# zendesk/min-tfs-client

Hardware: AMD Instinct MI355X
Metric: predict_req_per_s (higher is better)
Workload: dtype fp32; 1 GPU; model=identity-echo[resnet50], global_batch=32, parallelism=dp1, pipeline=4, encoding=turbo, grpc_impl=native, copy_mode=1, streaming=auto, transport=unix, servers_per_rank=1, gpu=True

## Files before the change

min_tfs_client_amd/ops/csrc/grpc_transport.cpp:

```cpp
#include <pybind11/eval.h>
#include <pybind11/functional.h>
#include <pybind11/pybind11.h>
#include <pybind11/stl.h>
#include <torch/extension.h>

#include <c10/hip/HIPCachingAllocator.h>
#include <c10/hip/HIPGuard.h>
#include <c10/hip/HIPStream.h>

#include <algorithm>
#include <atomic>
#include <chrono>
#include <condition_variable>
#include <cstring>
#include <deque>
#include <map>
#include <memory>
#include <mutex>
#include <set>
#include <string>
#include <thread>
#include <unordered_map>
#include <vector>

#include "h2core.h"
#include "hpack.h"
#include "staging.h"
#include "wire.h"

namespace py = pybind11;

namespace {

using h2::Buf;
using h2::Conn;
using h2::ConnError;
using h2::FrameHeader;

struct WireRegion {
  size_t offset;
  size_t nbytes;
  uintptr_t ptr;
  bool device;
};

void write_message_with_regions(Conn& conn, uint32_t stream,
                                const uint8_t* buf, size_t len,
                                const std::vector<WireRegion>& regions,
                                bool end_stream) {
  h2::DataMessageWriter w(conn, stream, len, end_stream);
  size_t pos = 0;
  for (const auto& r : regions) {
    if (r.offset < pos || r.nbytes > len || r.offset > len - r.nbytes)
      throw ConnError("bad streaming region");
    if (r.offset > pos) w.write(buf + pos, r.offset - pos);
    if (!r.device) {
      w.write(reinterpret_cast<const uint8_t*>(r.ptr), r.nbytes);
    } else {
      mi355x_staging::Lease lease;
      lease.ctx->d2h(reinterpret_cast<const void*>(r.ptr), r.nbytes,
                     [&w](const void* chunk, size_t n) {
                       w.write(static_cast<const uint8_t*>(chunk), n);
                     });
    }
    pos = r.offset + r.nbytes;
  }
  if (pos < len) w.write(buf + pos, len - pos);
  w.finish();
}

bool extract_streaming_reply(py::handle result,
                             std::unique_ptr<py::buffer_info>* info,
                             const uint8_t** buf, size_t* len,
                             std::vector<WireRegion>* regions) {
  if (!py::hasattr(result, "_wire_regions")) return false;
  py::object buffer = result.attr("buffer");
  *info = std::make_unique<py::buffer_info>(py::buffer(buffer).request());
  *buf = static_cast<const uint8_t*>((*info)->ptr);
  *len = size_t((*info)->size) * size_t((*info)->itemsize);
// ... 1306 lines not shown
    }
  }
};


class GrpcChannel {
 public:
  explicit GrpcChannel(const std::string& target,
                       std::string authority = "")
      : authority_(std::move(authority)) {
    if (authority_.empty()) {
      authority_ = target.rfind("unix:", 0) == 0 ? "localhost" : target;
    }
    int fd = h2::connect_target(target);
    conn_ = std::make_shared<Conn>(fd);
    h2::write_all(fd, reinterpret_cast<const uint8_t*>(h2::kPreface),
                  h2::kPrefaceLen);
    conn_->send_initial_settings();
    reader_ = std::thread([this] { reader_loop(); });
  }

  ~GrpcChannel() { close(); }

  void close() {
    bool was = closed_.exchange(true);
    if (was) return;
    conn_->mark_broken("channel closed");
    if (reader_.joinable()) reader_.join();
    fail_all_pending(GRPC_UNAVAILABLE, "channel closed");
  }

  uint32_t begin_stream(const std::string& path, double timeout_s) {
    auto p = std::make_shared<Pending>();
    uint32_t id;
    {
      std::unique_lock<std::mutex> lk(mu_);
      cv_.wait(lk, [&] {
        int64_t maxs;
        {
          std::lock_guard<std::mutex> flk(conn_->fc_mu);
          maxs = conn_->peer_max_streams;
          if (conn_->broken) return true;
        }
        return maxs < 0 || int64_t(pending_.size()) < maxs;
      });
      {
        std::lock_guard<std::mutex> flk(conn_->fc_mu);
        if (conn_->broken)
          throw RpcCallError(GRPC_UNAVAILABLE,
                             "channel broken: " + conn_->broken_why);
      }
      id = next_stream_;
      next_stream_ += 2;
      pending_[id] = p;
      conn_->open_send_stream(id);
      std::string block = make_request_headers(path, timeout_s);
      try {
        conn_->send_headers(id, block, false);
      } catch (const std::exception& e) {
        pending_.erase(id);
        conn_->close_send_stream(id);
        throw RpcCallError(GRPC_UNAVAILABLE, e.what());
      }
    }
    return id;
  }

  uint32_t start_call(const std::string& path, const uint8_t* data,
                      size_t len, double timeout_s) {
    uint32_t id = begin_stream(path, timeout_s);
    try {
      conn_->send_data_message(id, data, len, true);
    } catch (const std::exception& e) {
      std::lock_guard<std::mutex> lk(mu_);
      pending_.erase(id);
      conn_->close_send_stream(id);
      throw RpcCallError(GRPC_UNAVAILABLE, e.what());
    }
    return id;
  }

  hipStream_t device_stream(int dev) {
    return ProspectStreams::instance().get(dev);
  }

  uint32_t start_call_streaming(const std::string& path, const uint8_t* buf,
                                size_t len,
                                const std::vector<WireRegion>& regions,
                                double timeout_s, int parse_device = -1) {
    uint32_t id = begin_stream(path, timeout_s);
    if (parse_device >= 0) {
      hipStream_t ds = device_stream(parse_device);
      if (ds != nullptr) {
        auto p = find_pending(id);
        if (p) {
          std::lock_guard<std::mutex> lk(p->m);
          p->dparse.enabled = true;
          p->dparse.device = parse_device;
          p->dparse.stream = ds;
        }
      }
    }
    try {
      write_message_with_regions(*conn_, id, buf, len, regions, true);
    } catch (const std::exception& e) {
      std::lock_guard<std::mutex> lk(mu_);
// ... 21 lines not shown
    }
    auto quiesce = [&] {
      std::lock_guard<std::mutex> lk(p->m);
      if (p->dparse.enabled && p->dparse.stream != nullptr)
        (void)hipStreamSynchronize(p->dparse.stream);
    };
    std::unique_lock<std::mutex> lk(p->m);
    bool ok = true;
    if (timeout_s > 0) {
      ok = p->cv.wait_for(lk, std::chrono::duration<double>(timeout_s),
                          [&] { return p->done; });
    } else {
      p->cv.wait(lk, [&] { return p->done; });
    }
    if (!ok) {
      lk.unlock();
      quiesce();
      {
        std::lock_guard<std::mutex> glk(mu_);
        pending_.erase(id);
      }
      try {
        conn_->send_rst_stream(id, 8 );
      } catch (...) {
      }
      conn_->close_send_stream(id);
      cv_.notify_all();
      throw RpcCallError(GRPC_DEADLINE_EXCEEDED, "Deadline Exceeded");
    }
    ParsedResult r;
    r.resp = std::move(p->body.msg);
    int status = p->grpc_status;
    std::string msg = p->message;
    bool parsed = p->dparse.enabled && !p->dparse.failed && p->dparse.done;
    if (parsed) r.outs = std::move(p->dparse.outs);
    bool need_sync = p->dparse.enabled && p->dparse.stream != nullptr;
    hipStream_t ds = p->dparse.stream;
    lk.unlock();
    if (need_sync && hipStreamSynchronize(ds) != hipSuccess) parsed = false;
    if (parsed) record_consumer_stream(r.outs, r.outs.empty() ? 0 :
        r.outs.front().second.get_device());
    {
      std::lock_guard<std::mutex> glk(mu_);
      pending_.erase(id);
    }
    conn_->close_send_stream(id);
    cv_.notify_all();
    if (status != GRPC_OK)
      throw RpcCallError(status < 0 ? GRPC_INTERNAL : status, msg);
    r.parsed_ok = parsed;
    return r;
  }

  Buf wait(uint32_t id, double timeout_s) {
    std::shared_ptr<Pending> p;
    {
      std::lock_guard<std::mutex> lk(mu_);
      auto it = pending_.find(id);
      if (it == pending_.end())
        throw RpcCallError(GRPC_INTERNAL, "unknown call handle");
      p = it->second;
    }
    std::unique_lock<std::mutex> lk(p->m);
    bool ok = true;
    if (timeout_s > 0) {
      ok = p->cv.wait_for(lk, std::chrono::duration<double>(timeout_s),
                          [&] { return p->done; });
    } else {
      p->cv.wait(lk, [&] { return p->done; });
    }
    if (!ok) {
      lk.unlock();
      {
        std::lock_guard<std::mutex> glk(mu_);
        pending_.erase(id);
      }
      try {
        conn_->send_rst_stream(id, 8 );
      } catch (...) {
      }
      conn_->close_send_stream(id);
      cv_.notify_all();
      throw RpcCallError(GRPC_DEADLINE_EXCEEDED, "Deadline Exceeded");
    }
    Buf resp = std::move(p->body.msg);
    int status = p->grpc_status;
    std::string msg = p->message;
    lk.unlock();
    {
      std::lock_guard<std::mutex> glk(mu_);
      pending_.erase(id);
    }
    conn_->close_send_stream(id);
    cv_.notify_all();
    if (status != GRPC_OK)
      throw RpcCallError(status < 0 ? GRPC_INTERNAL : status, msg);
    return resp;
  }

 private:
  struct Pending {
    std::mutex m;
    std::condition_variable cv;
    bool done = false;
    int grpc_status = -1;
    std::string message;
    std::vector<h2::Header> resp_headers;
    HeaderBlock hb;
    MsgAssembly body;
    DeviceParse dparse;
  };

  std::shared_ptr<Conn> conn_;
  std::thread reader_;
  std::string authority_;
  std::atomic<bool> closed_{false};
  std::mutex mu_;
  std::condition_variable cv_;
  std::unordered_map<uint32_t, std::shared_ptr<Pending>> pending_;
  uint32_t next_stream_ = 1;

  std::string make_request_headers(const std::string& path,
                                   double timeout_s) {
    h2::HpackEncoder enc;
    std::string block;
    enc.add_indexed(&block, 3);
    enc.add_indexed(&block, 6);
    enc.add_literal(&block, 4, path, true);
    enc.add_literal(&block, 1, authority_);
    enc.add_literal(&block, "te", "trailers");
    enc.add_literal(&block, 31, "application/grpc");
    if (timeout_s > 0) {
      long ms = long(timeout_s * 1000.0);
      if (ms < 1) ms = 1;
      enc.add_literal(&block, "grpc-timeout", std::to_string(ms) + "m");
    }
    return block;
  }

  std::shared_ptr<Pending> find_pending(uint32_t id) {
    std::lock_guard<std::mutex> lk(mu_);
    auto it = pending_.find(id);
    return it == pending_.end() ? nullptr : it->second;
  }

  void complete(const std::shared_ptr<Pending>& p, int status,
                std::string msg) {
    {
      std::lock_guard<std::mutex> lk(p->m);
      if (p->done) return;
      p->grpc_status = status;
      p->message = std::move(msg);
      p->done = true;
    }
    p->cv.notify_all();
  }

  void fail_all_pending(int status, const std::string& msg) {
    std::vector<std::shared_ptr<Pending>> ps;
    {
      std::lock_guard<std::mutex> lk(mu_);
      for (auto& kv : pending_) ps.push_back(kv.second);
    }
    for (auto& p : ps) complete(p, status, msg);
    cv_.notify_all();
  }

  void process_headers(uint32_t stream, const std::shared_ptr<Pending>& p,
                       std::vector<h2::Header>&& headers, bool end_stream) {
    const std::string* gs = find_header(headers, "grpc-status");
    if (gs != nullptr || end_stream) {
      int status = GRPC_UNKNOWN;
      std::string msg = "missing grpc-status";
// ... 85 lines not shown
            break;
          }
          case h2::F_SETTINGS: {
            if (fh.flags & h2::FL_ACK) {
              h2::discard(conn_->fd, fh.length);
            } else {
              std::vector<uint8_t> payload(fh.length);
              if (fh.length)
                h2::read_full(conn_->fd, payload.data(), fh.length);
              conn_->apply_peer_settings(payload.data(), fh.length);
              conn_->send_settings_ack();
            }
            break;
          }
          case h2::F_PING: {
            uint8_t opaque[8];
            if (fh.length != 8) throw ConnError("bad PING");
            h2::read_full(conn_->fd, opaque, 8);
            if (!(fh.flags & h2::FL_ACK)) conn_->send_ping_ack(opaque);
            break;
          }
          case h2::F_WINDOW_UPDATE: {
            uint8_t buf4[4];
            if (fh.length != 4) throw ConnError("bad WINDOW_UPDATE");
            h2::read_full(conn_->fd, buf4, 4);
            conn_->apply_window_update(fh.stream,
                                       h2::be32(buf4) & 0x7fffffff);
            break;
          }
          case h2::F_RST_STREAM: {
            uint8_t buf4[4];
            if (fh.length != 4) throw ConnError("bad RST_STREAM");
            h2::read_full(conn_->fd, buf4, 4);
            auto p = find_pending(fh.stream);
            if (p)
              complete(p, GRPC_UNAVAILABLE,
                       "stream reset by server (http2 code " +
                           std::to_string(h2::be32(buf4)) + ")");
            break;
          }
          case h2::F_GOAWAY:
          default:
            h2::discard(conn_->fd, fh.length);
            break;
        }
      }
    } catch (const std::exception& e) {
      conn_->mark_broken(e.what());
      fail_all_pending(GRPC_UNAVAILABLE,
                       std::string("connection lost: ") + e.what());
    }
  }
};

}


PYBIND11_MODULE(_transport, m) {
  m.doc() = "Native gRPC (HTTP/2) transport for the MI355X serving stack";

  py::class_<OwnedBuf>(m, "OwnedBuf", py::buffer_protocol())
      .def_buffer([](OwnedBuf& b) -> py::buffer_info {
        return py::buffer_info(b.buf.p, 1,
                               py::format_descriptor<uint8_t>::format(),
                               1, {py::ssize_t(b.buf.len)}, {py::ssize_t(1)},
                               true );
      })
      .def("__len__", [](const OwnedBuf& b) { return b.buf.len; })
      .def("tobytes", [](const OwnedBuf& b) {
        return py::bytes(reinterpret_cast<const char*>(b.buf.p), b.buf.len);
      });

  static py::object rpc_error_cls = [&m]() {
    py::dict ns;
    py::exec(R"(
class NativeRpcError(Exception):
    """gRPC call failure from the native transport (code_int, details)."""
    def __init__(self, code, details):
        super().__init__(code, details)
        self.code_int = code
        self.details = details
)",
             ns, ns);
    py::object cls = ns["NativeRpcError"];
    m.attr("NativeRpcError") = cls;
    return cls;
  }();

  py::register_exception_translator([](std::exception_ptr ep) {
    try {
      if (ep) std::rethrow_exception(ep);
    } catch (const RpcCallError& e) {
      py::object exc = rpc_error_cls(e.code, e.what());
      PyErr_SetObject(rpc_error_cls.ptr(), exc.ptr());
    }
  });

  py::class_<GrpcServer>(m, "GrpcServer")
      .def(py::init<std::string, int>(), py::arg("address"),
           py::arg("workers") = 8)
      .def("start", &GrpcServer::start,
           py::call_guard<py::gil_scoped_release>())
      .def("register_handler", &GrpcServer::register_handler,
           py::arg("path"), py::arg("fn"))
      .def("register_handler_parsed", &GrpcServer::register_handler_parsed,
           py::arg("path"), py::arg("fn"), py::arg("device"),
// ... 107 lines not shown
            if (r.parsed_ok) {
              py::dict d;
              for (auto& kv : r.outs) d[py::str(kv.first)] = kv.second;
              outs = std::move(d);
            }
            return py::make_tuple(outs, OwnedBuf(std::move(r.resp)));
          },
          py::arg("id"), py::arg("timeout") = 0.0,
          "wait() for calls started with parse_device >= 0: returns "
          "({name: device tensor} | None, raw buf).")
      .def(
          "start_streaming",
          [](GrpcChannel& ch, const std::string& path, py::buffer data,
             py::list region_list, double timeout, int parse_device) {
            py::buffer_info info = data.request();
            const uint8_t* ptr = static_cast<const uint8_t*>(info.ptr);
            size_t len = size_t(info.size) * size_t(info.itemsize);
            std::vector<WireRegion> regions;
            regions.reserve(py::len(region_list));
            for (auto item : region_list) {
              auto t = py::reinterpret_borrow<py::tuple>(item);
              regions.push_back(WireRegion{
                  t[0].cast<size_t>(), t[1].cast<size_t>(),
                  uintptr_t(t[2].cast<uint64_t>()), t[3].cast<bool>()});
            }
            py::gil_scoped_release release;
            return ch.start_call_streaming(path, ptr, len, regions,
                                           timeout, parse_device);
          },
          py::arg("path"), py::arg("data"), py::arg("regions"),
          py::arg("timeout") = 0.0, py::arg("parse_device") = -1,
          "Streaming-region variant of start(); the send completes before "
          "this returns (region memory may be released), the response is "
          "collected with wait().")
      .def(
          "start",
          [](GrpcChannel& ch, const std::string& path, py::buffer data,
             double timeout) {
            py::buffer_info info = data.request();
            const uint8_t* ptr = static_cast<const uint8_t*>(info.ptr);
            size_t len = size_t(info.size) * size_t(info.itemsize);
            py::gil_scoped_release release;
            return ch.start_call(path, ptr, len, timeout);
          },
          py::arg("path"), py::arg("data"), py::arg("timeout") = 0.0)
      .def(
          "wait",
          [](GrpcChannel& ch, uint32_t id, double timeout) {
            py::gil_scoped_release release;
            Buf resp = ch.wait(id, timeout);
            return OwnedBuf(std::move(resp));
          },
          py::arg("id"), py::arg("timeout") = 0.0)
      .def("close", &GrpcChannel::close,
           py::call_guard<py::gil_scoped_release>());
}
```

min_tfs_client_amd/ops/csrc/native.cpp:

```cpp

#include <torch/extension.h>

#include <algorithm>
#include <atomic>
#include <chrono>
#include <cstring>
#include <string>
#include <thread>
#include <vector>

#include "wire.h"

namespace py = pybind11;

namespace mi355x {
at::Tensor cast_op(const at::Tensor& in, at::ScalarType out_dtype);
at::Tensor nchw_to_nhwc(const at::Tensor& in, at::ScalarType out_dtype);
at::Tensor nhwc_to_nchw(const at::Tensor& in, at::ScalarType out_dtype);
at::Tensor u8_nhwc_normalize(const at::Tensor& in, std::vector<double> scale,
                             std::vector<double> bias,
                             at::ScalarType out_dtype, bool out_nchw);
at::Tensor masked_mean_pool(const at::Tensor& hidden,
                            const c10::optional<at::Tensor>& mask,
                            bool normalize);
at::Tensor quantize_q8(const at::Tensor& in, double scale, double zp);
at::Tensor dequantize_q8(const at::Tensor& in, double scale, double zp);
void copy_device_to_host_ptr(const at::Tensor& src, void* dst, size_t n,
                             int mode);
void copy_host_ptr_to_device(const void* src, at::Tensor& dst, size_t n,
                             int mode);
bool hip_available();
}

namespace {

int torch_to_tf_dtype(at::ScalarType t) {
  switch (t) {
    case at::kFloat: return 1;
    case at::kDouble: return 2;
    case at::kInt: return 3;
    case at::kByte: return 4;
    case at::kShort: return 5;
    case at::kChar: return 6;
    case at::kComplexFloat: return 8;
    case at::kLong: return 9;
    case at::kBool: return 10;
    case at::kBFloat16: return 14;
    case at::kUInt16: return 17;
    case at::kComplexDouble: return 18;
    case at::kHalf: return 19;
    case at::kUInt32: return 22;
    case at::kUInt64: return 23;
    default:
      throw std::runtime_error("unsupported torch dtype for TensorProto");
  }
}

at::ScalarType tf_to_torch_dtype(int dt) {
  switch (dt) {
    case 1: return at::kFloat;
    case 2: return at::kDouble;
    case 3: return at::kInt;
    case 4: return at::kByte;
// ... 9 lines not shown
    case 22: return at::kUInt32;
    case 23: return at::kUInt64;
    default:
      throw std::runtime_error("unsupported TensorProto dtype " +
                               std::to_string(dt));
  }
}


py::bytes serialize_predict(bool is_request, const std::string& model_name,
                            int64_t version, const std::string& signature,
                            const std::vector<std::string>& names,
                            const std::vector<at::Tensor>& tensors,
                            int copy_mode) {
  TORCH_CHECK(names.size() == tensors.size(), "names/tensors mismatch");
  std::vector<tfswire::TensorMeta> metas(tensors.size());
  std::vector<at::Tensor> contig(tensors.size());
  for (size_t i = 0; i < tensors.size(); ++i) {
    contig[i] = tensors[i].contiguous();
    metas[i].dtype = torch_to_tf_dtype(contig[i].scalar_type());
    auto sizes = contig[i].sizes();
    metas[i].shape.assign(sizes.begin(), sizes.end());
    metas[i].content_bytes =
        uint64_t(contig[i].numel()) * contig[i].element_size();
    TORCH_CHECK(metas[i].content_bytes < (uint64_t(1) << 31),
                "tensor '", names[i], "' exceeds the 2GB tensor_content "
                "limit of the protobuf wire format");
  }
  auto plan = tfswire::plan_predict_message(is_request, model_name, version,
                                            signature, names, metas);
  PyObject* obj = PyBytes_FromStringAndSize(nullptr,
                                            Py_ssize_t(plan.total_size));
  if (!obj) throw std::bad_alloc();
  auto* buf = reinterpret_cast<uint8_t*>(PyBytes_AS_STRING(obj));
  tfswire::write_predict_message(buf, plan, is_request, model_name, version,
                                 signature, names, metas);
  {
    py::gil_scoped_release release;
    for (size_t i = 0; i < contig.size(); ++i) {
      const auto& span = plan.spans[i];
      if (span.nbytes == 0) continue;
      if (contig[i].is_cuda()) {
        mi355x::copy_device_to_host_ptr(contig[i], buf + span.offset,
                                        span.nbytes, copy_mode);
      } else {
        std::memcpy(buf + span.offset, contig[i].const_data_ptr(),
                    span.nbytes);
      }
    }
  }
  return py::reinterpret_steal<py::bytes>(obj);
}

constexpr size_t kStreamMinSpan = 64 * 1024;

py::tuple serialize_predict_streaming(bool is_request,
                                      const std::string& model_name,
                                      int64_t version,
                                      const std::string& signature,
                                      const std::vector<std::string>& names,
                                      const std::vector<at::Tensor>& tensors) {
  TORCH_CHECK(names.size() == tensors.size(), "names/tensors mismatch");
  std::vector<tfswire::TensorMeta> metas(tensors.size());
  std::vector<at::Tensor> contig(tensors.size());
  for (size_t i = 0; i < tensors.size(); ++i) {
    contig[i] = tensors[i].contiguous();
    metas[i].dtype = torch_to_tf_dtype(contig[i].scalar_type());
    auto sizes = contig[i].sizes();
    metas[i].shape.assign(sizes.begin(), sizes.end());
    metas[i].content_bytes =
        uint64_t(contig[i].numel()) * contig[i].element_size();
    TORCH_CHECK(metas[i].content_bytes < (uint64_t(1) << 31),
                "tensor '", names[i], "' exceeds the 2GB tensor_content "
                "limit of the protobuf wire format");
  }
  auto plan = tfswire::plan_predict_message(is_request, model_name, version,
                                            signature, names, metas);
  PyObject* obj = PyBytes_FromStringAndSize(nullptr,
                                            Py_ssize_t(plan.total_size));
  if (!obj) throw std::bad_alloc();
  auto* buf = reinterpret_cast<uint8_t*>(PyBytes_AS_STRING(obj));
  tfswire::write_predict_message(buf, plan, is_request, model_name, version,
                                 signature, names, metas);
  py::list regions;
  py::list keepalive;
  std::vector<size_t> order(contig.size());
  for (size_t i = 0; i < order.size(); ++i) order[i] = i;
  std::sort(order.begin(), order.end(), [&](size_t a, size_t b) {
    return plan.spans[a].offset < plan.spans[b].offset;
  });
  for (size_t idx : order) {
    const auto& span = plan.spans[idx];
    if (span.nbytes == 0) continue;
    const at::Tensor& t = contig[idx];
    if (t.is_cuda()) {
      regions.append(py::make_tuple(
          uint64_t(span.offset), uint64_t(span.nbytes),
          uint64_t(reinterpret_cast<uintptr_t>(t.const_data_ptr())), true));
      keepalive.append(t);
    } else if (span.nbytes >= kStreamMinSpan) {
      regions.append(py::make_tuple(
          uint64_t(span.offset), uint64_t(span.nbytes),
          uint64_t(reinterpret_cast<uintptr_t>(t.const_data_ptr())), false));
      keepalive.append(t);
    } else {
      std::memcpy(buf + span.offset, t.const_data_ptr(), span.nbytes);
    }
// ... 401 lines not shown
```

min_tfs_client_amd/ops/csrc/staging.h:

```cpp
#pragma once

#include <hip/hip_runtime_api.h>

#include <chrono>
#include <condition_variable>
#include <cstdint>
#include <cstdio>
#include <cstdlib>
#include <cstring>
#include <mutex>
#include <stdexcept>
#include <string>
#include <utility>
#include <vector>

namespace mi355x_staging {

#define MI355X_STAGING_CHECK(expr)                                       \
  do {                                                                   \
    hipError_t _e = (expr);                                              \
    if (_e != hipSuccess)                                                \
      throw std::runtime_error(std::string("HIP error in staging: ") +   \
                               hipGetErrorString(_e) + " at " #expr);    \
  } while (0)

inline size_t chunk_size() {
  static const size_t v = [] {
    const char* e = std::getenv("MI355X_STAGING_CHUNK");
    long long n = e ? std::atoll(e) : 0;
    if (n < (1 << 20) || n > (32 << 20)) n = 4 << 20;
    return size_t(n);
  }();
  return v;
}
constexpr int kMaxCtx = 8;

struct Ctx {
  hipStream_t stream = nullptr;
  void* buf[2] = {nullptr, nullptr};
  hipEvent_t evt[2] = {};
  hipEvent_t producer_evt = {};

  void init() {
    MI355X_STAGING_CHECK(
        hipStreamCreateWithFlags(&stream, hipStreamNonBlocking));
    for (int i = 0; i < 2; ++i) {
      MI355X_STAGING_CHECK(hipHostMalloc(&buf[i], chunk_size()));
      MI355X_STAGING_CHECK(
          hipEventCreateWithFlags(&evt[i], hipEventDisableTiming));
    }
    MI355X_STAGING_CHECK(
        hipEventCreateWithFlags(&producer_evt, hipEventDisableTiming));
  }

  void wait_producer(hipStream_t producer) {
    MI355X_STAGING_CHECK(hipEventRecord(producer_evt, producer));
    MI355X_STAGING_CHECK(hipStreamWaitEvent(stream, producer_evt, 0));
  }

  template <typename Consume>
  void d2h(const void* src_dev, size_t nbytes, Consume&& consume) {
    const size_t kChunk = chunk_size();
    size_t nchunks = (nbytes + kChunk - 1) / kChunk;
    const char* trace_path = std::getenv("MI355X_STAGING_TRACE");
    std::vector<double> wait_ms, consume_ms;
    size_t issued = 0;
    for (size_t c = 0; c < (nchunks < 2 ? nchunks : 2); ++c) {
      size_t off = c * kChunk;
      size_t len = nbytes - off < kChunk ? nbytes - off : kChunk;
      MI355X_STAGING_CHECK(hipMemcpyAsync(
          buf[c & 1], static_cast<const char*>(src_dev) + off, len,
          hipMemcpyDeviceToHost, stream));
      MI355X_STAGING_CHECK(hipEventRecord(evt[c & 1], stream));
      ++issued;
    }
    for (size_t c = 0; c < nchunks; ++c) {
      size_t off = c * kChunk;
      size_t len = nbytes - off < kChunk ? nbytes - off : kChunk;
      std::chrono::steady_clock::time_point t0, t1, t2;
      if (trace_path) t0 = std::chrono::steady_clock::now();
      MI355X_STAGING_CHECK(hipEventSynchronize(evt[c & 1]));
      if (trace_path) t1 = std::chrono::steady_clock::now();
      consume(static_cast<const void*>(buf[c & 1]), len);
      if (trace_path) {
        t2 = std::chrono::steady_clock::now();
        wait_ms.push_back(
            std::chrono::duration<double, std::milli>(t1 - t0).count());
        consume_ms.push_back(
            std::chrono::duration<double, std::milli>(t2 - t1).count());
      }
      if (issued < nchunks) {
        size_t noff = issued * kChunk;
        size_t nlen = nbytes - noff < kChunk ? nbytes - noff : kChunk;
        MI355X_STAGING_CHECK(hipMemcpyAsync(
            buf[issued & 1], static_cast<const char*>(src_dev) + noff, nlen,
            hipMemcpyDeviceToHost, stream));
        MI355X_STAGING_CHECK(hipEventRecord(evt[issued & 1], stream));
        ++issued;
      }
    }
    if (trace_path && !wait_ms.empty()) {
      FILE* f = std::fopen(trace_path, "a");
      if (f) {
        std::fprintf(f, "{\"nbytes\": %zu, \"chunks\": %zu, \"wait_ms\": [",
                     nbytes, nchunks);
        for (size_t i = 0; i < wait_ms.size(); ++i)
          std::fprintf(f, "%s%.4f", i ? "," : "", wait_ms[i]);
        std::fprintf(f, "], \"consume_ms\": [");
        for (size_t i = 0; i < consume_ms.size(); ++i)
          std::fprintf(f, "%s%.4f", i ? "," : "", consume_ms[i]);
        std::fprintf(f, "]}\n");
        std::fclose(f);
      }
    }
  }

  template <typename Produce>
  void h2d(void* dst_dev, size_t nbytes, Produce&& produce) {
    const size_t kChunk = chunk_size();
    size_t nchunks = (nbytes + kChunk - 1) / kChunk;
    for (size_t c = 0; c < nchunks; ++c) {
      size_t off = c * kChunk;
      size_t len = nbytes - off < kChunk ? nbytes - off : kChunk;
      if (c >= 2) MI355X_STAGING_CHECK(hipEventSynchronize(evt[c & 1]));
      produce(buf[c & 1], len);
      MI355X_STAGING_CHECK(hipMemcpyAsync(
          static_cast<char*>(dst_dev) + off, buf[c & 1], len,
          hipMemcpyHostToDevice, stream));
      MI355X_STAGING_CHECK(hipEventRecord(evt[c & 1], stream));
    }
    MI355X_STAGING_CHECK(hipStreamSynchronize(stream));
  }
};

class Pool {
 public:
  static Pool& instance() {
    static Pool pool;
    return pool;
  }

  Ctx* acquire() {
    std::unique_lock<std::mutex> lk(mu_);
    cv_.wait(lk, [this] { return !free_.empty() || created_ < kMaxCtx; });
    if (!free_.empty()) {
      Ctx* c = free_.back();
      free_.pop_back();
      return c;
    }
    ++created_;
    lk.unlock();
    auto* c = new Ctx();
    try {
      c->init();
    } catch (...) {
      delete c;
      std::lock_guard<std::mutex> lk2(mu_);
      --created_;
      cv_.notify_one();
      throw;
    }
    return c;
  }

  void release(Ctx* c) {
    {
      std::lock_guard<std::mutex> lk(mu_);
      free_.push_back(c);
    }
    cv_.notify_one();
  }

 private:
  std::mutex mu_;
  std::condition_variable cv_;
  std::vector<Ctx*> free_;
  int created_ = 0;
};

struct Lease {
  Ctx* ctx;
  Lease() : ctx(Pool::instance().acquire()) {}
  ~Lease() { Pool::instance().release(ctx); }
  Lease(const Lease&) = delete;
  Lease& operator=(const Lease&) = delete;
};

}
```

min_tfs_client_amd/turbo.py:

```python
from __future__ import annotations

import os
from typing import Dict, Optional, Union

import grpc

try:
    import torch
except ImportError:
    torch = None

from .ops import require_native
from .utils.allocator import tune_malloc
from .utils.metrics import MetricsRegistry
from .utils.tracing import trace_span

_PREDICT_PATH = "/tensorflow.serving.PredictionService/Predict"

_CHANNEL_OPTS = [
    ("grpc.max_send_message_length", 1 << 30),
    ("grpc.max_receive_message_length", 1 << 30),
    ("grpc.http2.max_frame_size", 16 * 1024 * 1024 - 1),
]

# ... 166 lines not shown
        targets = [target] if isinstance(target, str) else list(target)
        n = max(len(targets), max(1, num_channels))
        self._channels = []
        self._stubs = []
        if backend == "native":
            if credentials is not None:
                raise ValueError("backend='native' is cleartext (h2c); use "
                                 "backend='grpcio' for TLS")
            from . import _transport
            for i in range(n):
                ch = _transport.GrpcChannel(targets[i % len(targets)])
                self._channels.append(ch)
                self._stubs.append(_NativeStub(ch, _PREDICT_PATH))
        elif backend == "grpcio":
            opts = _CHANNEL_OPTS + (options or [])
            for i in range(n):
                copts = opts + [("grpc.use_local_subchannel_pool", 1),
                                ("grpc.channel_id", i)]
                tgt = targets[i % len(targets)]
                if credentials:
                    ch = grpc.secure_channel(tgt, credentials,
                                             options=copts)
                else:
                    ch = grpc.insecure_channel(tgt, options=copts)
                self._channels.append(ch)
                self._stubs.append(ch.unary_unary(
                    _PREDICT_PATH, request_serializer=_identity,
                    response_deserializer=_identity))
        else:
            raise ValueError(f"unknown backend {backend!r}")
        self._channel = self._channels[0]
        self._predict = self._stubs[0]
        self._rr = 0
        self.metrics = MetricsRegistry()
        self.__send_pool = None

    @property
    def _send_pool(self):
        if self.__send_pool is None:
            from concurrent.futures import ThreadPoolExecutor
            self.__send_pool = ThreadPoolExecutor(
                max_workers=16, thread_name_prefix="turbo-send")
        return self.__send_pool

    def _next_stub(self):
        stub = self._stubs[self._rr % len(self._stubs)]
        self._rr += 1
        return stub

    def close(self):
        if self.__send_pool is not None:
            self.__send_pool.shutdown(wait=False)
            self.__send_pool = None
        for ch in self._channels:
            ch.close()

    def __enter__(self):
        return self

    def __exit__(self, *exc):
        self.close()

    def serialize_request(self, model_name: str,
                          inputs: Dict[str, "torch.Tensor"],
                          model_version: Optional[int] = None,
                          signature_name: str = "",
                          copy_mode: int = 1) -> bytes:
        names = list(inputs.keys())
        tensors = [inputs[k] for k in names]
        return self._native.serialize_predict_request(
            model_name, -1 if model_version is None else model_version,
            signature_name, names, tensors, copy_mode)

    def _serialize_streaming(self, model_name, inputs, model_version,
                             signature_name):
        names = list(inputs.keys())
        tensors = [inputs[k] for k in names]
        blob, regions, keepalive = self._native.serialize_predict_streaming(
            True, model_name,
            -1 if model_version is None else model_version,
            signature_name, names, tensors)
        if torch is not None and any(r[3] for r in regions):
            torch.cuda.current_stream().synchronize()
        return blob, regions, keepalive

    def predict(self, model_name: str, inputs: Dict[str, "torch.Tensor"],
                timeout: float = 60.0,
                model_version: Optional[int] = None,
                signature_name: str = "",
                output_device: Optional[Union[str, "torch.device"]] = None,
                copy_mode: int = 1,
                zero_copy: bool = False,
                transform: Optional[Dict[str, tuple]] = None,
                streaming: Optional[bool] = None
                ) -> Dict[str, "torch.Tensor"]:
        if transform:
            inputs = dict(inputs)
            for name, (layout, dtype) in transform.items():
                t = inputs[name]
                if t.is_cuda:
                    from . import ops
                    if layout == "nhwc":
                        inputs[name] = ops.nchw_to_nhwc(t, dtype or t.dtype)
                    elif layout == "nchw":
                        inputs[name] = ops.nhwc_to_nchw(t, dtype or t.dtype)
                    elif dtype is not None and dtype != t.dtype:
# ... 65 lines not shown
        if TurboPredictClient._TF_TO_TORCH is None:
            from .constants import ENUM_TO_TF_MAPPING
            TurboPredictClient._TF_TO_TORCH = {
                enum: TF_TO_TORCH_MAPPING[name]
                for enum, name in ENUM_TO_TF_MAPPING.items()
                if name in TF_TO_TORCH_MAPPING}
        _spec, spans, _filt = self._native.parse_predict_spans(resp, False)
        out = {}
        for d in spans:
            if d is None:
                _s, full, _ = self._native.parse_predict_response(
                    resp, "cpu", 1)
                return full
            dtype = TurboPredictClient._TF_TO_TORCH[d["dtype"]]
            mv = memoryview(resp)[d["offset"]:d["offset"] + d["nbytes"]]
            with warnings.catch_warnings():
                warnings.simplefilter("ignore")
                t = torch.frombuffer(mv, dtype=dtype)
            out[d["name"]] = t.reshape(d["shape"])
        return out

    def predict_sharded(self, model_name: str,
                        inputs: Dict[str, "torch.Tensor"],
                        shards: int = 2,
                        timeout: float = 60.0,
                        model_version: Optional[int] = None,
                        signature_name: str = "",
                        output_device: Optional[str] = None,
                        copy_mode: int = 1,
                        streaming: Optional[bool] = None
                        ) -> Dict[str, "torch.Tensor"]:
        if shards <= 1 or len(self._stubs) < 2:
            return self.predict(model_name, inputs, timeout, model_version,
                                signature_name, output_device, copy_mode,
                                streaming=streaming)
        keys = list(inputs.keys())
        if any(inputs[k].dim() == 0 for k in keys):
            return self.predict(model_name, inputs, timeout, model_version,
                                signature_name, output_device, copy_mode,
                                streaming=streaming)
        batch = inputs[keys[0]].shape[0]
        if any(inputs[k].shape[0] != batch for k in keys) \
                or batch < shards:
            return self.predict(model_name, inputs, timeout, model_version,
                                signature_name, output_device, copy_mode,
                                streaming=streaming)
        base, rem = divmod(batch, shards)
        sizes = [base + (1 if i < rem else 0) for i in range(shards)]
        use_streaming = (self.backend == "native" if streaming is None
                         else streaming)
        if use_streaming and self.backend != "native":
            raise ValueError("streaming=True requires backend='native'")

        shard_views = []
        off = 0
        for n in sizes:
            shard_views.append({k: inputs[k].narrow(0, off, n)
                                for k in keys})
            off += n

        dev = str(output_device) if output_device is not None else "cpu"
        parse_dev = -1
        if (use_streaming and dev.startswith("cuda") and torch is not None
                and os.environ.get("MI355X_RX_PARSE", "1") != "0"):
            parse_dev = torch.device(dev).index or 0

        def send_shard(i):
            shard = shard_views[i]
            stub = self._stubs[i % len(self._stubs)]
            if use_streaming:
                blob, regions, keepalive = self._serialize_streaming(
                    model_name, shard, model_version, signature_name)
                if parse_dev >= 0:
                    return stub.future_streaming_parsed(
                        blob, regions, parse_dev, timeout)
                return stub.future_streaming(blob, regions, timeout)
            blob = self.serialize_request(model_name, shard, model_version,
                                          signature_name, copy_mode)
            return stub.future(blob, timeout)

        if self.backend == "native" and shards > 1:
            sends = [self._send_pool.submit(send_shard, i)
                     for i in range(shards)]
            futs = [s.result() for s in sends]
        else:
            futs = [send_shard(i) for i in range(shards)]
        parts = []
        try:
            for fut in futs:
                if isinstance(fut, _NativeParsedFuture):
                    outs, raw = fut.result_parsed()
                    if outs is None:
                        _s, outs, _ = self._native.parse_predict_response(
                            raw, dev, copy_mode)
                    parts.append(outs)
                else:
                    _s, outputs, _ = self._native.parse_predict_response(
                        fut.result(), dev, copy_mode)
                    parts.append(outputs)
        except Exception:
            for fut in futs:
                fut.cancel()
            raise
        merged = {}
        for k in parts[0]:
            vals = [p[k] for p in parts]
            if isinstance(vals[0], torch.Tensor) and vals[0].dim() > 0:
                merged[k] = torch.cat(vals, dim=0)
            else:
                merged[k] = vals[0]
        return merged

    def predict_future(self, model_name, inputs, timeout=60.0,
                       model_version=None, signature_name="",
                       copy_mode: int = 1):
        if self.backend == "native":
            blob, regions, keepalive = self._serialize_streaming(
                model_name, inputs, model_version, signature_name)
            fut = self._next_stub().future_streaming(blob, regions, timeout)
            del keepalive
        else:
            blob = self.serialize_request(model_name, inputs, model_version,
                                          signature_name, copy_mode)
            fut = self._next_stub().future(blob, timeout)

        def decode(resp_bytes, output_device="cpu"):
            _s, outputs, _ = self._native.parse_predict_response(
                resp_bytes, str(output_device), copy_mode)
            return outputs

        return fut, decode
```

Measured before the change: 702.2 req/s.

## Move sharded predict fan-out into native C++ with a sender thread pool

Adds a native predict_sharded entry that plans each shard's PredictRequest, synchronizes producer streams once, sends shards in parallel on a persistent C++ sender pool over rotating channels, and merges device-parsed outputs with at::cat. All of this happens behind one GIL release. The aim is to remove Python-level per-shard serialization, executor dispatch and GIL contention. It also adds tracing counters and a streams_started property, and it creates a process-wide thread pool.

```diff
diff --git a/min_tfs_client_amd/ops/csrc/grpc_transport.cpp b/min_tfs_client_amd/ops/csrc/grpc_transport.cpp
--- a/min_tfs_client_amd/ops/csrc/grpc_transport.cpp
+++ b/min_tfs_client_amd/ops/csrc/grpc_transport.cpp
@@ -25,6 +25,7 @@
 
 #include "h2core.h"
 #include "hpack.h"
+#include "sharded.h"
 #include "staging.h"
 #include "wire.h"
 
@@ -1437,6 +1438,7 @@
       }
       id = next_stream_;
       next_stream_ += 2;
+      streams_started_.fetch_add(1, std::memory_order_relaxed);
       pending_[id] = p;
       conn_->open_send_stream(id);
       std::string block = make_request_headers(path, timeout_s);
@@ -1564,6 +1566,10 @@
     return r;
   }
 
+  uint64_t streams_started() const {
+    return streams_started_.load(std::memory_order_relaxed);
+  }
+
   Buf wait(uint32_t id, double timeout_s) {
     std::shared_ptr<Pending> p;
     {
@@ -1631,6 +1637,7 @@
   std::condition_variable cv_;
   std::unordered_map<uint32_t, std::shared_ptr<Pending>> pending_;
   uint32_t next_stream_ = 1;
+  std::atomic<uint64_t> streams_started_{0};
 
   std::string make_request_headers(const std::string& path,
                                    double timeout_s) {
@@ -1822,6 +1829,285 @@
     }
   }
 };
+
+
+inline int scalar_to_tf_dtype(at::ScalarType t) {
+  switch (t) {
+    case at::kFloat: return 1;
+    case at::kDouble: return 2;
+    case at::kInt: return 3;
+    case at::kByte: return 4;
+    case at::kShort: return 5;
+    case at::kChar: return 6;
+    case at::kComplexFloat: return 8;
+    case at::kLong: return 9;
+    case at::kBool: return 10;
+    case at::kBFloat16: return 14;
+    case at::kUInt16: return 17;
+    case at::kComplexDouble: return 18;
+    case at::kHalf: return 19;
+    case at::kUInt32: return 22;
+    case at::kUInt64: return 23;
+    default:
+      throw std::invalid_argument("unsupported torch dtype for TensorProto");
+  }
+}
+
+class SenderPool {
+ public:
+  static SenderPool& instance() {
+    static SenderPool* pool = new SenderPool();
+    return *pool;
+  }
+
+  bool submit(std::function<void()> job) {
+    {
+      std::lock_guard<std::mutex> lk(mu_);
+      if (stopping_) return false;
+      if (threads_.empty())
+        for (int i = 0; i < tfsshard::kSenderPoolSize; ++i)
+          threads_.emplace_back([this] { loop(); });
+      queue_.push_back(std::move(job));
+    }
+    cv_.notify_one();
+    return true;
+  }
+
+  void shutdown() {
+    std::vector<std::thread> threads;
+    {
+      std::lock_guard<std::mutex> lk(mu_);
+      if (threads_.empty()) return;
+      stopping_ = true;
+      threads.swap(threads_);
+    }
+    cv_.notify_all();
+    for (auto& t : threads)
+      if (t.joinable()) t.join();
+    std::lock_guard<std::mutex> lk(mu_);
+    stopping_ = false;
+  }
+
+ private:
+  void loop() {
+    for (;;) {
+      std::function<void()> job;
+      {
+        std::unique_lock<std::mutex> lk(mu_);
+        cv_.wait(lk, [this] { return stopping_ || !queue_.empty(); });
+        if (queue_.empty()) return;
+        job = std::move(queue_.front());
+        queue_.pop_front();
+      }
+      job();
+    }
+  }
+
+  std::mutex mu_;
+  std::condition_variable cv_;
+  std::deque<std::function<void()>> queue_;
+  std::vector<std::thread> threads_;
+  bool stopping_ = false;
+};
+
+std::atomic<uint32_t> g_shard_rotation{0};
+
+inline double ms_since(std::chrono::steady_clock::time_point t0) {
+  return std::chrono::duration<double, std::milli>(
+             std::chrono::steady_clock::now() - t0)
+      .count();
+}
+
+struct ShardedCall {
+  struct Shard {
+    tfsshard::ShardPlan plan;
+    std::vector<WireRegion> regions;
+    GrpcChannel* ch = nullptr;
+    std::atomic<bool> claimed{false};
+    bool started = false;
+    uint32_t id = 0;
+    std::exception_ptr err;
+    double send_start_ms = 0.0, send_ms = 0.0;
+  };
+
+  std::string path;
+  double timeout = 0.0;
+  int parse_device = -1;
+  std::chrono::steady_clock::time_point t0;
+  std::vector<Shard> shards;
+  std::mutex m;
+  std::condition_variable cv;
+  size_t sends_pending = 0;
+
+  explicit ShardedCall(size_t n) : shards(n), sends_pending(n) {}
+
+  bool try_send(size_t i) {
+    Shard& s = shards[i];
+    if (s.claimed.exchange(true)) return false;
+    s.send_start_ms = ms_since(t0);
+    try {
+      s.id = s.ch->start_call_streaming(path, s.plan.skeleton.get(),
+                                        s.plan.size, s.regions,
+                                        timeout, parse_device);
+      s.started = true;
+    } catch (...) {
+      s.err = std::current_exception();
+    }
+    s.send_ms = ms_since(t0) - s.send_start_ms;
+    std::lock_guard<std::mutex> lk(m);
+    --sends_pending;
+    cv.notify_all();
+    return true;
+  }
+
+  void wait_sends() {
+    std::unique_lock<std::mutex> lk(m);
+    cv.wait(lk, [this] { return sends_pending == 0; });
+  }
+};
+
+struct ShardedResult {
+  bool merged = false;
+  std::vector<std::pair<std::string, at::Tensor>> outs;
+  std::vector<GrpcChannel::ParsedResult> parts;
+};
+
+ShardedResult run_predict_sharded(
+    const std::vector<GrpcChannel*>& channels, const std::string& path,
+    const std::string& model_name, int64_t version,
+    const std::string& signature, const std::vector<std::string>& names,
+    const std::vector<tfsshard::Input>& inputs,
+    const std::vector<int>& input_devices, int shards, int parse_device,
+    double timeout) {
+  static const char* trace_path = std::getenv("MI355X_SHARDED_TRACE");
+  const auto t0 = std::chrono::steady_clock::now();
+  const size_t n = size_t(shards);
+  auto call = std::make_shared<ShardedCall>(n);
+  call->path = path;
+  call->timeout = timeout;
+  call->parse_device = parse_device;
+  call->t0 = t0;
+
+  const auto sizes = tfsshard::shard_sizes(inputs[0].shape[0], shards);
+  const uint32_t n_ch = uint32_t(channels.size());
+  const uint32_t start =
+      tfsshard::next_start_channel(g_shard_rotation, n_ch, uint32_t(shards));
+  int64_t row = 0;
+  for (size_t i = 0; i < n; ++i) {
+    auto& s = call->shards[i];
+    s.plan = tfsshard::plan_shard(model_name, version, signature, names,
+                                  inputs, row, sizes[i]);
+    row += sizes[i];
+    s.regions.reserve(s.plan.regions.size());
+    for (const auto& r : s.plan.regions)
+      s.regions.push_back(WireRegion{r.offset, r.nbytes, r.ptr, r.device});
+    s.ch = channels[tfsshard::shard_channel(start, uint32_t(i), n_ch)];
+  }
+  const double plan_ms = ms_since(t0);
+
+  for (int dev : input_devices) {
+    hipStream_t cur = c10::hip::getCurrentHIPStream(
+                          static_cast<c10::DeviceIndex>(dev))
+                          .stream();
+    if (hipStreamSynchronize(cur) != hipSuccess)
+      throw RpcCallError(GRPC_INTERNAL,
+                         "producer stream synchronize failed");
+  }
+  const double sync_ms = ms_since(t0) - plan_ms;
+
+  for (size_t i = 1; i < n; ++i)
+    (void)SenderPool::instance().submit([call, i] { call->try_send(i); });
+  for (size_t i = 0; i < n; ++i) call->try_send(i);
+  call->wait_sends();
+  const double sends_done_ms = ms_since(t0);
+
+  ShardedResult res;
+  res.parts.resize(n);
+  std::exception_ptr first_err;
+  for (size_t i = 0; i < n; ++i) {
+    auto& s = call->shards[i];
+    if (!s.started) {
+      if (!first_err) first_err = s.err;
+      continue;
+    }
+    double remaining = 0.0;
+    if (timeout > 0) {
+      remaining = timeout - ms_since(t0) * 1e-3;
+      if (remaining < 1e-3) remaining = 1e-3;
+    }
+    try {
+      if (parse_device >= 0) {
+        res.parts[i] = s.ch->wait_parsed(s.id, remaining);
+      } else {
+        res.parts[i].resp = s.ch->wait(s.id, remaining);
+      }
+    } catch (...) {
+      if (!first_err) first_err = std::current_exception();
+    }
+  }
+  const double wait_ms = ms_since(t0) - sends_done_ms;
+  if (first_err) {
+    res.parts.clear();
+    try {
+      std::rethrow_exception(first_err);
+    } catch (const RpcCallError&) {
+      throw;
+    } catch (const std::exception& e) {
+      throw RpcCallError(GRPC_INTERNAL, e.what());
+    }
+  }
+
+  const auto t_merge = std::chrono::steady_clock::now();
+  bool all_parsed = parse_device >= 0;
+  for (auto& p : res.parts) all_parsed = all_parsed && p.parsed_ok;
+  if (all_parsed) {
+    const auto& first = res.parts[0].outs;
+    for (auto& p : res.parts) {
+      all_parsed = all_parsed && p.outs.size() == first.size();
+      for (size_t k = 0; all_parsed && k < first.size(); ++k)
+        all_parsed = p.outs[k].first == first[k].first;
+    }
+  }
+  if (all_parsed) {
+    const auto& first = res.parts[0].outs;
+    for (size_t k = 0; k < first.size(); ++k) {
+      if (first[k].second.dim() == 0) {
+        res.outs.emplace_back(first[k].first, first[k].second);
+        continue;
+      }
+      std::vector<at::Tensor> pieces;
+      pieces.reserve(n);
+      for (auto& p : res.parts) pieces.push_back(p.outs[k].second);
+      res.outs.emplace_back(first[k].first, at::cat(pieces, 0));
+    }
+    res.merged = true;
+    res.parts.clear();
+  }
+
+  if (trace_path) {
+    std::string line = "{\"shards\": " + std::to_string(n) +
+                       ", \"start_channel\": " + std::to_string(start) +
+                       ", \"plan_ms\": " + std::to_string(plan_ms) +
+                       ", \"sync_ms\": " + std::to_string(sync_ms) +
+                       ", \"send_start_ms\": [";
+    for (size_t i = 0; i < n; ++i)
+      line += (i ? "," : "") + std::to_string(call->shards[i].send_start_ms);
+    line += "], \"send_ms\": [";
+    for (size_t i = 0; i < n; ++i)
+      line += (i ? "," : "") + std::to_string(call->shards[i].send_ms);
+    line += "], \"sends_done_ms\": " + std::to_string(sends_done_ms) +
+            ", \"wait_ms\": " + std::to_string(wait_ms) +
+            ", \"merge_ms\": " + std::to_string(ms_since(t_merge)) +
+            ", \"merged\": " + (res.merged ? "true" : "false") +
+            ", \"total_ms\": " + std::to_string(ms_since(t0)) + "}\n";
+    FILE* f = std::fopen(trace_path, "a");
+    if (f) {
+      std::fputs(line.c_str(), f);
+      std::fclose(f);
+    }
+  }
+  return res;
+}
 
 }
 
@@ -2035,6 +2321,94 @@
             return OwnedBuf(std::move(resp));
           },
           py::arg("id"), py::arg("timeout") = 0.0)
+      .def_property_readonly(
+          "streams_started", &GrpcChannel::streams_started,
+          "Number of streams (calls) opened on this channel so far.")
       .def("close", &GrpcChannel::close,
            py::call_guard<py::gil_scoped_release>());
+
+  m.def(
+      "predict_sharded",
+      [](const std::vector<GrpcChannel*>& channels, const std::string& path,
+         const std::string& model_name, int64_t version,
+         const std::string& signature,
+         const std::vector<std::string>& names,
+         const std::vector<at::Tensor>& tensors, int shards,
+         int parse_device, double timeout) -> py::object {
+        if (channels.empty()) throw py::value_error("no channels");
+        for (auto* ch : channels)
+          if (ch == nullptr) throw py::value_error("channel is None");
+        if (names.size() != tensors.size() || tensors.empty())
+          throw py::value_error("names/tensors mismatch");
+        if (shards < 1) throw py::value_error("shards must be >= 1");
+        std::vector<at::Tensor> contig(tensors.size());
+        std::vector<tfsshard::Input> inputs(tensors.size());
+        std::vector<int> input_devices;
+        for (size_t i = 0; i < tensors.size(); ++i) {
+          const at::Tensor& t = tensors[i];
+          if (t.dim() == 0)
+            throw py::value_error("sharded inputs need a batch dimension");
+          if (!t.is_cuda() && !t.is_cpu())
+            throw py::value_error("inputs must be CPU or GPU tensors");
+          if (t.size(0) != tensors[0].size(0))
+            throw py::value_error("inputs disagree on the dim-0 size");
+          contig[i] = t.contiguous();
+          auto& in = inputs[i];
+          in.dtype = scalar_to_tf_dtype(contig[i].scalar_type());
+          auto sz = contig[i].sizes();
+          in.shape.assign(sz.begin(), sz.end());
+          in.elem_size = size_t(contig[i].element_size());
+          in.data = static_cast<const uint8_t*>(contig[i].const_data_ptr());
+          in.device = contig[i].is_cuda();
+          if (in.device) {
+            int dev = int(contig[i].get_device());
+            if (std::find(input_devices.begin(), input_devices.end(), dev) ==
+                input_devices.end())
+              input_devices.push_back(dev);
+          }
+        }
+        if (tensors[0].size(0) < shards)
+          throw py::value_error("batch is smaller than the shard count");
+        ShardedResult r;
+        {
+          py::gil_scoped_release release;
+          r = run_predict_sharded(channels, path, model_name, version,
+                                  signature, names, inputs, input_devices,
+                                  shards, parse_device, timeout);
+        }
+        if (r.merged) {
+          py::dict d;
+          for (auto& kv : r.outs) d[py::str(kv.first)] = kv.second;
+          return std::move(d);
+        }
+        py::list parts;
+        for (auto& p : r.parts) {
+          py::object outs = py::none();
+          if (p.parsed_ok) {
+            py::dict d;
+            for (auto& kv : p.outs) d[py::str(kv.first)] = kv.second;
+            outs = std::move(d);
+          }
+          parts.append(py::make_tuple(outs, OwnedBuf(std::move(p.resp))));
+        }
+        return std::move(parts);
+      },
+      py::arg("channels"), py::arg("path"), py::arg("model_name"),
+      py::arg("version"), py::arg("signature"), py::arg("names"),
+      py::arg("tensors"), py::arg("shards"), py::arg("parse_device") = -1,
+      py::arg("timeout") = 0.0,
+      "One logical Predict split along dim 0 into `shards` PredictRequests "
+      "sent in parallel over distinct channels (rotating between "
+      "requests), behind a single GIL release. Returns the merged "
+      "{name: device tensor} dict when every shard was device-parsed, "
+      "else the per-shard [(outs | None, raw buf), ...] list.");
+
+  m.def(
+      "shutdown_sender_pool", [] { SenderPool::instance().shutdown(); },
+      py::call_guard<py::gil_scoped_release>(),
+      "Drain and join the sharded-send thread pool (restarted lazily by "
+      "the next sharded call).");
+  m.attr("SENDER_POOL_SIZE") = tfsshard::kSenderPoolSize;
+  py::module_::import("atexit").attr("register")(
+      m.attr("shutdown_sender_pool"));
 }
diff --git a/min_tfs_client_amd/ops/csrc/native.cpp b/min_tfs_client_amd/ops/csrc/native.cpp
--- a/min_tfs_client_amd/ops/csrc/native.cpp
+++ b/min_tfs_client_amd/ops/csrc/native.cpp
@@ -9,6 +9,7 @@
 #include <thread>
 #include <vector>
 
+#include "sharded.h"
 #include "wire.h"
 
 namespace py = pybind11;
@@ -124,7 +125,7 @@
   return py::reinterpret_steal<py::bytes>(obj);
 }
 
-constexpr size_t kStreamMinSpan = 64 * 1024;
+using tfsshard::kStreamMinSpan;
 
 py::tuple serialize_predict_streaming(bool is_request,
                                       const std::string& model_name,
diff --git a/min_tfs_client_amd/ops/csrc/sharded.h b/min_tfs_client_amd/ops/csrc/sharded.h
--- /dev/null
+++ b/min_tfs_client_amd/ops/csrc/sharded.h
@@ -0,0 +1,115 @@
+#pragma once
+
+#include <atomic>
+#include <cstdint>
+#include <cstring>
+#include <memory>
+#include <stdexcept>
+#include <string>
+#include <vector>
+
+#include "wire.h"
+
+namespace tfsshard {
+
+constexpr size_t kStreamMinSpan = 64 * 1024;
+
+constexpr int kSenderPoolSize = 8;
+
+inline std::vector<int64_t> shard_sizes(int64_t batch, int shards) {
+  if (shards < 1 || batch < shards)
+    throw std::invalid_argument("shard_sizes: need 1 <= shards <= batch");
+  const int64_t base = batch / shards;
+  const int64_t rem = batch % shards;
+  std::vector<int64_t> sizes(static_cast<size_t>(shards));
+  for (int i = 0; i < shards; ++i)
+    sizes[size_t(i)] = base + (i < rem ? 1 : 0);
+  return sizes;
+}
+
+struct Input {
+  int dtype = 0;
+  std::vector<int64_t> shape;
+  size_t elem_size = 0;
+  const uint8_t* data = nullptr;
+  bool device = false;
+
+  uint64_t row_bytes() const {
+    uint64_t n = elem_size;
+    for (size_t d = 1; d < shape.size(); ++d) n *= uint64_t(shape[d]);
+    return n;
+  }
+};
+
+struct Region {
+  size_t offset;
+  size_t nbytes;
+  uintptr_t ptr;
+  bool device;
+};
+
+struct ShardPlan {
+  std::unique_ptr<uint8_t[]> skeleton;
+  size_t size = 0;
+  std::vector<Region> regions;
+};
+
+inline ShardPlan plan_shard(const std::string& model_name, int64_t version,
+                            const std::string& signature,
+                            const std::vector<std::string>& names,
+                            const std::vector<Input>& inputs,
+                            int64_t row_off, int64_t rows) {
+  if (names.size() != inputs.size())
+    throw std::invalid_argument("plan_shard: names/inputs mismatch");
+  std::vector<tfswire::TensorMeta> metas(inputs.size());
+  for (size_t i = 0; i < inputs.size(); ++i) {
+    const Input& in = inputs[i];
+    if (in.shape.empty() || row_off < 0 || rows < 0 ||
+        row_off + rows > in.shape[0])
+      throw std::invalid_argument("plan_shard: rows out of range for '" +
+                                  names[i] + "'");
+    metas[i].dtype = in.dtype;
+    metas[i].shape = in.shape;
+    metas[i].shape[0] = rows;
+    metas[i].content_bytes = uint64_t(rows) * in.row_bytes();
+    if (metas[i].content_bytes >= (uint64_t(1) << 31))
+      throw std::invalid_argument(
+          "tensor '" + names[i] + "' exceeds the 2GB tensor_content limit "
+          "of the protobuf wire format");
+  }
+  auto plan = tfswire::plan_predict_message(true, model_name, version,
+                                            signature, names, metas);
+  ShardPlan out;
+  out.size = size_t(plan.total_size);
+  out.skeleton.reset(new uint8_t[out.size ? out.size : 1]);
+  tfswire::write_predict_message(out.skeleton.get(), plan, true, model_name,
+                                 version, signature, names, metas);
+  for (size_t i = 0; i < inputs.size(); ++i) {
+    const auto& span = plan.spans[i];
+    if (span.nbytes == 0) continue;
+    const uint8_t* src =
+        inputs[i].data + uint64_t(row_off) * inputs[i].row_bytes();
+    if (inputs[i].device || span.nbytes >= kStreamMinSpan) {
+      out.regions.push_back(Region{size_t(span.offset), size_t(span.nbytes),
+                                   reinterpret_cast<uintptr_t>(src),
+                                   inputs[i].device});
+    } else {
+      std::memcpy(out.skeleton.get() + span.offset, src, span.nbytes);
+    }
+  }
+  return out;
+}
+
+inline uint32_t next_start_channel(std::atomic<uint32_t>& counter,
+                                   uint32_t n_channels, uint32_t shards) {
+  if (n_channels == 0) throw std::invalid_argument("no channels");
+  uint32_t k = counter.fetch_add(1, std::memory_order_relaxed);
+  return uint32_t((uint64_t(k) * shards) % n_channels);
+}
+
+inline uint32_t shard_channel(uint32_t start, uint32_t shard,
+                              uint32_t n_channels) {
+  return (start + shard) % n_channels;
+}
+
+}
diff --git a/min_tfs_client_amd/ops/csrc/staging.h b/min_tfs_client_amd/ops/csrc/staging.h
--- a/min_tfs_client_amd/ops/csrc/staging.h
+++ b/min_tfs_client_amd/ops/csrc/staging.h
@@ -40,6 +40,7 @@
   void* buf[2] = {nullptr, nullptr};
   hipEvent_t evt[2] = {};
   hipEvent_t producer_evt = {};
+  double acquire_ms = 0.0;
 
   void init() {
     MI355X_STAGING_CHECK(
@@ -102,8 +103,9 @@
     if (trace_path && !wait_ms.empty()) {
       FILE* f = std::fopen(trace_path, "a");
       if (f) {
-        std::fprintf(f, "{\"nbytes\": %zu, \"chunks\": %zu, \"wait_ms\": [",
-                     nbytes, nchunks);
+        std::fprintf(f, "{\"nbytes\": %zu, \"chunks\": %zu, "
+                     "\"acquire_ms\": %.4f, \"wait_ms\": [",
+                     nbytes, nchunks, acquire_ms);
         for (size_t i = 0; i < wait_ms.size(); ++i)
           std::fprintf(f, "%s%.4f", i ? "," : "", wait_ms[i]);
         std::fprintf(f, "], \"consume_ms\": [");
@@ -180,7 +182,17 @@
 
 struct Lease {
   Ctx* ctx;
-  Lease() : ctx(Pool::instance().acquire()) {}
+  Lease() {
+    if (std::getenv("MI355X_STAGING_TRACE") == nullptr) {
+      ctx = Pool::instance().acquire();
+      return;
+    }
+    auto t0 = std::chrono::steady_clock::now();
+    ctx = Pool::instance().acquire();
+    ctx->acquire_ms = std::chrono::duration<double, std::milli>(
+                          std::chrono::steady_clock::now() - t0)
+                          .count();
+  }
   ~Lease() { Pool::instance().release(ctx); }
   Lease(const Lease&) = delete;
   Lease& operator=(const Lease&) = delete;
diff --git a/min_tfs_client_amd/turbo.py b/min_tfs_client_amd/turbo.py
--- a/min_tfs_client_amd/turbo.py
+++ b/min_tfs_client_amd/turbo.py
@@ -242,6 +242,9 @@
         if self.__send_pool is not None:
             self.__send_pool.shutdown(wait=False)
             self.__send_pool = None
+        if self.backend == "native":
+            from . import _transport
+            _transport.shutdown_sender_pool()
         for ch in self._channels:
             ch.close()
 
@@ -413,18 +416,24 @@
         if use_streaming and self.backend != "native":
             raise ValueError("streaming=True requires backend='native'")
 
+        dev = str(output_device) if output_device is not None else "cpu"
+        parse_dev = -1
+        if (use_streaming and dev.startswith("cuda") and torch is not None
+                and os.environ.get("MI355X_RX_PARSE", "1") != "0"):
+            parse_dev = torch.device(dev).index or 0
+
+        if (use_streaming and torch is not None
+                and os.environ.get("MI355X_NATIVE_SHARDED", "1") != "0"):
+            return self._predict_sharded_native(
+                model_name, keys, inputs, shards, timeout, model_version,
+                signature_name, dev, parse_dev, copy_mode)
+
         shard_views = []
         off = 0
         for n in sizes:
             shard_views.append({k: inputs[k].narrow(0, off, n)
                                 for k in keys})
             off += n
-
-        dev = str(output_device) if output_device is not None else "cpu"
-        parse_dev = -1
-        if (use_streaming and dev.startswith("cuda") and torch is not None
-                and os.environ.get("MI355X_RX_PARSE", "1") != "0"):
-            parse_dev = torch.device(dev).index or 0
 
         def send_shard(i):
             shard = shard_views[i]
@@ -472,6 +481,35 @@
                 merged[k] = vals[0]
         return merged
 
+    @_translate_native_error
+    def _predict_sharded_native(self, model_name, keys, inputs, shards,
+                                timeout, model_version, signature_name,
+                                dev, parse_dev, copy_mode):
+        from . import _transport
+        with trace_span("turbo.sharded_native", model=model_name,
+                        shards=shards):
+            res = _transport.predict_sharded(
+                self._channels, _PREDICT_PATH, model_name,
+                -1 if model_version is None else model_version,
+                signature_name, keys, [inputs[k] for k in keys], shards,
+                parse_dev, timeout or 0.0)
+        if isinstance(res, dict):
+            return res
+        parts = []
+        for outs, raw in res:
+            if outs is None:
+                _s, outs, _ = self._native.parse_predict_response(
+                    raw, dev, copy_mode)
+            parts.append(outs)
+        merged = {}
+        for k in parts[0]:
+            vals = [p[k] for p in parts]
+            if isinstance(vals[0], torch.Tensor) and vals[0].dim() > 0:
+                merged[k] = torch.cat(vals, dim=0)
+            else:
+                merged[k] = vals[0]
+        return merged
+
     def predict_future(self, model_name, inputs, timeout=60.0,
                        model_version=None, signature_name="",
                        copy_mode: int = 1):
```

Measured after the change: 808.2 req/s (median of 6 runs). 1.15x the previous value.
